# bgrozev/libjitsi

Measured on AMD Instinct MI355X. Metric: SRTP protect+unprotect packets/s + GB/s, 1200B AES_CM_128_HMAC_SHA1_80, 1-8 GPU, higher is better.
Workload: dtype u8; 1 GPU; configs[1]: 10k concurrent SSRCs x 1200-B RTP, AES_CM_128_HMAC_SHA1_80, protect + unprotect per step; ssrcs_per_gpu=10000, pkt_len=1200, region_align=16, ssrc_mix=round-robin, keysets=1, parallelism=ssrc-sharded x1 (one process per GPU), stream_events=device

## Files before the change

### libjitsi_amd/_native.py

```python
from __future__ import annotations

import ctypes as C
import os

import numpy as np

_HERE = os.path.dirname(os.path.abspath(__file__))
LIB_PATH = os.environ.get("SRTP_MI355X_LIB") or os.path.join(_HERE, "libsrtp_mi355x.so")
HEADER_PATH = os.path.join(os.path.dirname(_HERE), "include", "srtp_mi355x.h")

NULL_ENCRYPTION, AESCM_ENCRYPTION, AESF8_ENCRYPTION, TWOFISH_ENCRYPTION, TWOFISHF8_ENCRYPTION = range(5)
AESGCM_ENCRYPTION = 5
PROFILE_AEAD_AES_128_GCM, PROFILE_AEAD_AES_256_GCM = 0x0007, 0x0008
NULL_AUTHENTICATION, HMACSHA1_AUTHENTICATION = 0, 1
KIND_RTP, KIND_RTCP = 0, 1
(STATUS_OK, STATUS_DROP_REPLAY, STATUS_DROP_AUTH, STATUS_DROP_VERSION, STATUS_DROP_NO_CONTEXT,
 STATUS_ERR_CAPACITY, STATUS_ERR_MALFORMED, STATUS_DROP_INVALID, STATUS_NOT_PROCESSED,
 STATUS_SKIPPED, STATUS_ERR_INTERNAL) = range(11)
STATUS_NAMES = ["OK", "DROP_REPLAY", "DROP_AUTH", "DROP_VERSION", "DROP_NO_CONTEXT",
                "ERR_CAPACITY", "ERR_MALFORMED", "DROP_INVALID", "NOT_PROCESSED", "SKIPPED",
                "ERR_INTERNAL"]
NUM_STATUS = len(STATUS_NAMES)
DEBUG_FORCE_CHAIN_STALL = 0x1
DEBUG_FORCE_WIDE = 0x2
# ... 19 lines not shown
    "srtp_engine_last_error", "srtp_factory_create", "srtp_factory_close",
    "srtp_transformer_create", "srtp_transformer_set_factory", "srtp_transformer_close",
    "srtp_transform_device", "srtp_transform_host", "srtp_engine_sync",
    "srtp_get_context_state", "srtp_engine_num_contexts", "srtp_engine_set_timing",
    "srtp_engine_read_timing", "srtp_derive_session_keys", "srtp_export_contexts",
    "srtp_set_context_state", "srtp_pipeline_create", "srtp_pipeline_destroy",
    "srtp_pipeline_slot_get", "srtp_pipeline_submit", "srtp_pipeline_wait",
    "srtp_engine_stats", "srtp_engine_stream", "srtp_shard_of", "srtp_dispatch_plan", "srtp_dispatch_create",
    "srtp_dispatch_destroy", "srtp_dispatch_last_error", "srtp_dispatch_num_shards",
    "srtp_dispatch_engine", "srtp_dispatch_factory_create", "srtp_dispatch_factory_close",
    "srtp_dispatch_transformer_create", "srtp_dispatch_transformer_set_factory",
    "srtp_dispatch_transformer_close", "srtp_dispatch_transform_host", "srtp_dispatch_submit_host",
    "srtp_dispatch_wait_host",
    "srtp_dispatch_get_context_state", "srtp_dispatch_set_context_state", "srtp_dispatch_stats",
    "srtp_tls_export_keying_material", "srtp_dtls_profile_keys", "srtp_dtls_transformer_create",
    "srtp_engine_get_opts", "srtp_derive_session_keys_n", "srtp_derive_session_keys_for",
    "srtp_block_encrypt", "srtp_aes_gcm", "srtp_aggregator_opts_default", "srtp_aggregator_create",
    "srtp_aggregator_submit", "srtp_aggregator_flush", "srtp_aggregator_stats",
    "srtp_aggregator_destroy", "srtp_derive_session_keys_auth", "srtp_skein512_mac",
    "srtp_engine_set_debug", "srtp_contexts_save", "srtp_contexts_restore",
    "srtp_dispatch_route", "srtp_aggregator_create_dispatch", "srtp_transformer_info",
    "srtp_rawpacket_batch_create", "srtp_rawpacket_batch_create_dispatch",
    "srtp_rawpacket_batch_destroy", "srtp_rawpacket_transform", "srtp_rawpacket_result",
    "srtp_dispatch_host_times", "srtp_pipeline_submit_ex", "srtp_aggregator_transform",
    "srtp_aggregator_transformer_info", "srtp_rawpacket_transform_one", "srtp_device_count",
    "srtp_host_register", "srtp_host_unregister", "srtp_host_is_registered", "srtp_pipeline_submit_host",
    "srtp_pipeline_submit_gather",
    "srtp_pipeline_create_ex", "srtp_host_alloc", "srtp_host_free",
    "srtp_queue_create", "srtp_queue_submit", "srtp_queue_reap", "srtp_queue_outstanding",
    "srtp_queue_aggregator", "srtp_queue_destroy", "srtp_queue_release", "srtp_packet_may_throw",
    "srtp_rawpacket_batch_set_aggregator", "srtp_rawpacket_submit", "srtp_rawpacket_complete",
    "srtp_pipeline_query", "srtp_aes_gcm_device",
    "srtp_engine_enable_aead", "srtp_gcm_packet_job", "srtp_dtls_profile_keys_ex",
    "srtp_dispatch_enable_aead",
    "srtp_aes_gcm_device_ex", "srtp_gf128_mul", "srtp_gcm_hpowers", "srtp_gcm_wave_max",
    "srtp_small_aead_max",
    "srtp_trailer_room", "srtp_engine_trailer_room", "srtp_aggregator_trailer_room",
    "srtp_engine_gcm_stats", "srtp_dispatch_gcm_stats", "srtp_gcm_open_lane_min", "srtp_gcm_open_wave_min",
    "srtp_gcm_open_wave_max",
    "srtp_gcm_spec_ok", "srtp_gcm_fix_action",
    "srtp_fanout_device", "srtp_fanout_host", "srtp_engine_fanout_stats", "srtp_fanout_job",
    "srtp_fanout_device_rw", "srtp_fanout_host_rw", "srtp_fanout_rewrite_job",
    "srtp_fanout_device_ast", "srtp_fanout_host_ast", "srtp_fanout_ast_job",
    "srtp_fanout_device_pay", "srtp_fanout_host_pay", "srtp_fanout_pay_job",
    "srtp_transform_device_lvl", "srtp_transform_host_lvl", "srtp_engine_audio_level_stats",
    "srtp_audio_level_job",
    "srtp_fanout_device_red", "srtp_fanout_host_red", "srtp_engine_fanout_red_stats", "srtp_fanout_red_job",
    "srtp_fanout_device_fec", "srtp_fanout_host_fec", "srtp_engine_fanout_fec_stats", "srtp_fanout_fec_job",
]
STAGES = ["parse", "sort", "verify", "walk", "protect", "decrypt"]


KERNEL_SOURCES = ["srtp_kernels.hip", "aes_rounds_asm.inc", "srtp_kernels.h", "srtp_types.h", "engine.cpp",
                  "gcm_job.h", "fanout_job.h", "bundle_plan.h", "audio_level_job.h", "red_job.h", "fec_job.h"]


def kernel_source_sha16() -> str:
    import hashlib
    h = hashlib.sha256()
    for name in KERNEL_SOURCES:
        with open(os.path.join(_HERE, "csrc", name), "rb") as f:
            h.update(f.read())
    return h.hexdigest()[:16]


class SrtpError(RuntimeError):
    pass


class Policy(C.Structure):
    _fields_ = [(n, C.c_int32) for n in (
        "enc_type", "enc_key_len", "auth_type", "auth_key_len", "auth_tag_len", "salt_key_len")]


class EngineOpts(C.Structure):
    _fields_ = [("device", C.c_int32), ("check_replay", C.c_int32),
                ("abort_on_error", C.c_int32), ("max_contexts", C.c_uint32),
                ("max_factories", C.c_uint32), ("max_transformers", C.c_uint32),
                ("max_batch", C.c_uint32)]


class CtxState(C.Structure):
    _fields_ = [("roc", C.c_int32), ("s_l", C.c_int32), ("seq_num_set", C.c_int32),
                ("guessed_roc", C.c_int32), ("sent_index", C.c_int32),
                ("received_index", C.c_int32), ("replay_window", C.c_uint64),
                ("key_set", C.c_uint32)]


class Stats(C.Structure):
    _fields_ = ([("bundles", C.c_uint64), ("packets", C.c_uint64),
                 ("status", C.c_uint64 * NUM_STATUS)] +
                [(n, C.c_uint64) for n in ("roc_rechecks", "repaired", "ctx_overflow", "ctx_live",
                                           "ctx_tombstones", "ctx_slots", "rehashes", "chain_stalls", "long_walked",
                                           "holes", "small_bundles", "small_aead_bundles")])

    def as_dict(self) -> dict:
        d = {k: getattr(self, k) for k, _ in self._fields_ if k != "status"}
        d["status"] = {STATUS_NAMES[i]: int(self.status[i]) for i in range(NUM_STATUS)}
        return d


class DtlsKeys(C.Structure):
    _fields_ = [("srtp", Policy), ("srtcp", Policy), ("key_len", C.c_int32),
                ("salt_len", C.c_int32), ("keying_material_len", C.c_int32),
                ("client_key", C.c_uint8 * 16), ("server_key", C.c_uint8 * 16),
                ("client_salt", C.c_uint8 * 14), ("server_salt", C.c_uint8 * 14)]

# ... 358 lines not shown
```

### libjitsi_amd/csrc/srtp_kernels.hip

```cpp
#include <hip/hip_runtime.h>
#include <stdlib.h>
#include <string.h>

#include <algorithm>
#include <atomic>


#include "../../include/srtp_mi355x.h"
#include "audio_level_job.h"
#include "fanout_job.h"
#include "fec_job.h"
#include "gcm_job.h"
#include "red_job.h"
#include "srtp_kernels.h"

namespace srtp {

__device__ uint32_t d_te0[256];

constexpr int kBlock = 256;

__device__ __forceinline__ uint32_t rotl(uint32_t x, uint32_t n) {
    return __builtin_amdgcn_alignbit(x, x, 32u - n);
}
__device__ __forceinline__ uint32_t bswap(uint32_t x) { return __builtin_bswap32(x); }

__device__ __forceinline__ uint32_t ld_u8(const uint8_t *p) { return *p; }
__device__ __forceinline__ uint32_t ld_be32(const uint8_t *p) {
    return (ld_u8(p) << 24) | (ld_u8(p + 1) << 16) | (ld_u8(p + 2) << 8) | ld_u8(p + 3);
}

__device__ __forceinline__ uint64_t mix64(uint64_t x) {
    x ^= x >> 30; x *= 0xbf58476d1ce4e5b9ull;
    x ^= x >> 27; x *= 0x94d049bb133111ebull;
    x ^= x >> 31;
    return x;
}

__device__ __forceinline__ int32_t java_ishl1(int32_t n) { return (int32_t)(1u << (n & 31)); }
__device__ __forceinline__ int64_t java_lshl(int64_t v, int64_t n) {
    return (int64_t)((uint64_t)v << (n & 63));
}

constexpr int kTeWords = 32768;
constexpr int kTeCounters = 16;
constexpr int kAesBlock = 1024;
constexpr int kMacBlock = 256;
#ifndef SRTP_UNPROTECT_BLOCK
#define SRTP_UNPROTECT_BLOCK 1024
#endif
#ifndef SRTP_PROTECT_BLOCK
#define SRTP_PROTECT_BLOCK 1024
#endif
constexpr int kUnprotectBlock = SRTP_UNPROTECT_BLOCK;
constexpr int kProtectBlock = SRTP_PROTECT_BLOCK;

__device__ __forceinline__ void fill_te4(uint32_t *s_te) {
    const int W = (int)(blockDim.x >> 6), w = (int)(threadIdx.x >> 6), lane = (int)(threadIdx.x & 63u);
    const uint32_t r = (uint32_t)(lane >> 5) << 3;
    for (int j0 = 0; w + j0 * W < 256; j0 += 64) {
        const int ej = w + (j0 + lane) * W;
        const uint32_t mine = ej < 256 ? d_te0[ej] : 0u;
        for (int k = 0; k < 64; k++) {
            const int e = w + (j0 + k) * W;
            if (e >= 256) break;
            const uint32_t v = __builtin_amdgcn_readlane(mine, k);
            s_te[(e << 6) | lane] = rotl(v, r);
// ... 1932 lines not shown
    c.enc = ks->enc_type; c.auth = ks->auth_type; c.T = ks->tag_len; c.kind = ks->kind;
    c.check_replay = a.check_replay != 0;
    c.reverse = REV;
    const int32_t tid = (int32_t)(a.ctx_keys[slot] >> 32);
    const bool mac = c.auth != SRTP_NULL_AUTHENTICATION;
    uint32_t i = i0;
    uint32_t walked = 0u;
    for (;;) {
        const WalkRec *R = sm.rec;
        const uint32_t *G0 = sm.g0, *OK = sm.ok;
        int nvalid;
        if (pw) {
            const uint32_t jb = i - pw->base;
            int nv = 0;
#pragma unroll
            for (int k = 0; k < kLongPer; k++) {
                const uint32_t t = jb + (uint32_t)(lane + 64 * k);
                nv += (t < pw->win && pw->key[t] == key) ? 1 : 0;
            }
            nvalid = (int)__reduce_add_sync(~0ull, (unsigned)nv);
            R = pw->rec + jb; G0 = pw->g0 + jb; OK = pw->ok + jb;
        } else {
            int nv = 0;
#pragma unroll
            for (int k = 0; k < kLongPer; k++) {
                const int j = lane + 64 * k;
                const uint32_t idx = i + (uint32_t)j;
                const bool v = idx < a.n && a.sk_out[idx] == key;
                uint4 r = make_uint4(0u, 0u, 0u, 0u);
                if (v) r = reinterpret_cast<const uint4 *>(a.sv_out)[idx];
                reinterpret_cast<uint4 *>(sm.rec)[j] = r;
                if (REV) {
                    const uint32_t p = r.x & kRecIdxMask;
                    const uint2 go = v ? gok_of(a, p) : make_uint2(0u, 0u);
                    sm.g0[j] = go.x;
                    sm.ok[j] = go.y;
                }
                nv += v ? 1 : 0;
            }
            nvalid = (int)__reduce_add_sync(~0ull, (unsigned)nv);
            walk_sync();
        }
        if (nvalid == 0) break;
        int f = 0;
        if (c.kind == SRTP_KIND_RTP && (st.flags & 1u)) {
            const int p0 = lane * kLongPer;
            int32_t lsum = 0;
#pragma unroll 1
            for (int r = 0; r < kLongPer; r++) {
                const int pos = p0 + r;
                if (pos >= nvalid) break;
                const int32_t seq = (int32_t)(R[pos].word & 0xffffu);
                const int32_t sl = pos ? (int32_t)(R[pos - 1].word & 0xffffu) : st.b;
                int32_t d;
                if (sl < 32768) d = (seq - sl > 32768) ? -1 : 0;
                else d = (sl - 32768 > seq) ? 1 : 0;
                lsum += d;
            }
            uint32_t roc = (uint32_t)st.a + (uint32_t)wave_excl_scan(lsum);
            int first_bad = kLongPer;
#pragma unroll 1
            for (int r = 0; r < kLongPer; r++) {
                const int pos = p0 + r;
                if (pos >= nvalid) { first_bad = min(first_bad, r); break; }
                const WalkRec rec = R[pos];
                const int32_t seq = (int32_t)(rec.word & 0xffffu);
                const int32_t sl = pos ? (int32_t)(R[pos - 1].word & 0xffffu) : st.b;
                const uint32_t roc_prev = roc;
                int32_t d;
                if (sl < 32768) d = (seq - sl > 32768) ? -1 : 0;
                else d = (sl - 32768 > seq) ? 1 : 0;
                roc += (uint32_t)d;
                const int64_t delta = (java_lshl((int64_t)(int32_t)roc, 16) | (int64_t)seq) -
                                      (java_lshl((int64_t)(int32_t)roc_prev, 16) | (int64_t)sl);
                const int L = (int)(rec.lc & 0xffffu), C = (int)(rec.lc >> 16);
                bool g = delta > 0;
                if (REV) {
                    const int newL = mac ? (L - c.T > 0 ? L - c.T : 0) : L;
                    if (!(rec.p & kRecSkipDec)) g = g && !enc_would_throw(c.enc, rec.h, newL - rec.h);
                    if (g && mac) {
                        const uint32_t g0 = G0[pos], okb = OK[pos];
                        if (roc == g0) {
                            g = (okb & 1u) != 0u;
                        } else if ((okb & 4u) && roc == g0 - 1u) {
                            g = (okb & 2u) != 0u;
                        } else {
                            const uint32_t p = rec.p & kRecIdxMask;
                            ReverifyArgs rv;
                            rv.pkt = a.seg + a.off[p];
                            rv.mid = a.mid + 5 * (size_t)p;
                            rv.tailc = (a.spec[p] & kSpecDid) ? a.tailc + 16 * (size_t)p : nullptr;
                            g = reverify_tag<SK>(a, rv, ks, L, (int32_t)roc);
                        }
                    }
                } else {
                    g = g && L + (mac ? c.T : 0) <= C && !enc_would_throw(c.enc, rec.h, L - rec.h);
                }
                sm.roc[pos] = roc;
                sm.info[pos] = (g ? 1u : 0u) | ((uint32_t)((uint64_t)delta & 63u) << 1);
                if (!g) { first_bad = r; break; }
            }
            const unsigned long long bad_lanes = __ballot(first_bad < kLongPer);
            f = nvalid;
            if (bad_lanes) {
                const int bl = __ffsll((long long)bad_lanes) - 1;
                f = min(f, bl * kLongPer + __builtin_amdgcn_readlane(first_bad, bl));
            }
            int32_t dsum = 0;
            uint32_t recheck = 0u;
#pragma unroll 1
            for (int r = 0; r < kLongPer; r++) {
                const int pos = p0 + r;
                if (pos >= f) break;
                const WalkRec rec = R[pos];
                const uint32_t p = rec.p & kRecIdxMask;
                const int L = (int)(rec.lc & 0xffffu);
                const uint32_t rr = sm.roc[pos];
                a.w_cw[p] = rr;
                a.w_len[p] = (uint32_t)(REV ? (mac ? (L - c.T > 0 ? L - c.T : 0) : L) : L + (mac ? c.T : 0));
                a.w_status[p] = SRTP_STATUS_OK;
                if (REV && mac) {
                    const uint32_t g0 = G0[pos], okb = OK[pos];
                    if (rr != g0 && !((okb & 4u) && rr == g0 - 1u)) recheck++;
                }
                dsum += (int32_t)(sm.info[pos] >> 1);
            }
            if (f > 0) {
// ... 5 lines not shown
                    const int pos = p0 + r;
                    if (pos >= f) break;
                    after -= (int32_t)(sm.info[pos] >> 1);
                    if (after < 64) bits |= 1ull << after;
                }
                bits = wave_or64(bits);
                st.window = (total < 64 ? st.window << total : 0ull) | bits;
                st.a = (int32_t)sm.roc[f - 1];
                st.b = (int32_t)(R[f - 1].word & 0xffffu);
                st.g = st.a;
                const uint32_t rc = (uint32_t)__reduce_add_sync(~0ull, recheck);
                if (lane == 0 && rc) atomicAdd(&a.counters[kCtrRocRecheck], (unsigned long long)rc);
            }
        }
        walked += (uint32_t)(f < nvalid ? (c.kind == SRTP_KIND_RTP ? 1 : nvalid - f) : 0);
        if (f < nvalid) {
            const int stop = c.kind == SRTP_KIND_RTP ? f + 1 : nvalid;
            if (lane == 0) {
                for (int k = f; k < stop; k++) {
                    const WalkRec r = R[k];
                    uint32_t g0 = 0u, ok = 0u;
                    if (REV) { g0 = G0[k]; ok = OK[k]; }
                    (void)walk_one<SK>(a, ks, c, st, r, g0, ok, false, tid);
                }
            }
            bcast_state(st);
            i += (uint32_t)stop;
        } else {
            i += (uint32_t)nvalid;
        }
        walk_sync();
        if (nvalid < kLongStep && f >= nvalid) break;
    }
    if (lane == 0) {
        a.ctx[slot] = st;
        atomicAdd(&a.counters[kCtrLongWalked], (unsigned long long)walked);
    }
}

constexpr int kWalkBlock = 64;
#ifndef SRTP_WALK_PER
#define SRTP_WALK_PER 4
#endif
constexpr int kWalkPer = SRTP_WALK_PER;
constexpr int kWalkSpan = kWalkBlock * kWalkPer;
constexpr int kWalkAhead = 256;
constexpr int kWalkWin = kWalkSpan + kWalkAhead;
#ifndef SRTP_MED_MIN
#define SRTP_MED_MIN 32
#endif
constexpr uint32_t kMedMin = SRTP_MED_MIN;
constexpr int kMedMax = kWalkSpan / SRTP_MED_MIN + 1;
static_assert(kMedMax <= 64, "one medium chain start per lane");

constexpr int kChainPer = kWalkSpan / kWalkBlock;
static_assert(kLongMin == (uint32_t)kWalkSpan, "a long chain reaches the end of the tile it starts in");

struct ChainAgg {
    int32_t dsum;
    uint32_t x;
    uint32_t tshift;
    uint64_t bits;
    int32_t s_l;
    bool hasx, broken;
};
struct ChainState {
    uint32_t roc;
    int32_t s_l;
    uint64_t window;
    bool broken;
    bool stalled = false;
};

__device__ __forceinline__ ChainState chain_apply(ChainState p, const ChainAgg &g) {
    if (p.broken || g.broken || (g.hasx && p.roc != g.x) ||
        (int64_t)(int32_t)p.roc + g.dsum > (int64_t)0x7fffffff) {
        p.broken = true;
        return p;
    }
    p.roc += (uint32_t)g.dsum;
    p.s_l = g.s_l;
    p.window = (g.tshift < 64u ? p.window << g.tshift : 0ull) | g.bits;
    return p;
}

__device__ __forceinline__ ChainAgg chain_compose(const ChainAgg &g1, const ChainAgg &g2) {
    ChainAgg o;
    o.broken = g1.broken || g2.broken ||
               (g1.hasx && g2.hasx && g2.x - (uint32_t)g1.dsum != g1.x);
    o.dsum = g1.dsum + g2.dsum;
    o.hasx = g1.hasx || g2.hasx;
    o.x = g1.hasx ? g1.x : g2.x - (uint32_t)g1.dsum;
    o.tshift = min(g1.tshift + g2.tshift, 64u);
    o.bits = (g2.tshift < 64u ? g1.bits << g2.tshift : 0ull) | g2.bits;
    o.s_l = g2.s_l;
    return o;
}

constexpr int kLinkWords = 10;
__device__ __forceinline__ void gran_put(uint64_t *p, uint32_t epoch, uint32_t v) {
    __hip_atomic_store(p, ((uint64_t)v << 32) | epoch, __ATOMIC_RELAXED, __HIP_MEMORY_SCOPE_AGENT);
}
__device__ __forceinline__ bool gran_get(const uint64_t *p, uint32_t epoch, uint32_t &v) {
    const uint64_t g = __hip_atomic_load(p, __ATOMIC_RELAXED, __HIP_MEMORY_SCOPE_AGENT);
    v = (uint32_t)(g >> 32);
    return (uint32_t)g == epoch;
// ... 129 lines not shown
__device__ __forceinline__ void chain_window(const uint32_t m[kChainPer], int f, uint32_t &tshift,
                                             uint64_t &bits) {
    const int lane = (int)(threadIdx.x & 63u);
    int32_t msum = 0;
#pragma unroll
    for (int r = 0; r < kChainPer; r++)
        if (lane * kChainPer + r < f) msum += (int32_t)m[r];
    const int32_t total = (int32_t)__reduce_add_sync(~0ull, (unsigned)msum);
    int32_t after = total - wave_excl_scan(msum);
    uint64_t b = 0ull;
#pragma unroll
    for (int r = 0; r < kChainPer; r++) {
        if (lane * kChainPer + r < f) {
            after -= (int32_t)m[r];
            if (after < 64) b |= 1ull << after;
        }
    }
    bits = wave_or64(b);
    tshift = (uint32_t)min(total, 64);
}

struct ChainFix {
    uint32_t i0;
    CtxState st;
};

template <bool REV>
__device__ __forceinline__ ChainFix chain_part(const BundleArgs &a, uint32_t tile, uint32_t epoch, uint32_t base, uint32_t j0,
                               int n, bool head, bool out, int32_t prev_seq_in, const WalkRec *s_rec,
                               const uint32_t *s_g0, const uint32_t *s_ok) {
    ChainFix fix;
    fix.i0 = kNoSlot;
    const int lane = (int)(threadIdx.x & 63u);
    const uint32_t slot = a.sk_out[base + j0];
    const CtxState st0 = a.ctx[slot];
    const KeySet *ks = a.keysets + st0.ks;
    WalkCtx c;
    c.enc = ks->enc_type; c.auth = ks->auth_type; c.T = ks->tag_len; c.kind = ks->kind;
    const bool mac = c.auth != SRTP_NULL_AUTHENTICATION;
    const int32_t prev_seq = head ? st0.b : prev_seq_in;
    int32_t dpre[kChainPer];
    uint32_t m[kChainPer], xr[kChainPer];
    int32_t seqv[kChainPer];
    bool lok[kChainPer];
    int32_t lsum = 0;
#pragma unroll
    for (int r = 0; r < kChainPer; r++) {
        const int pos = lane * kChainPer + r;
        dpre[r] = 0; m[r] = 0u; xr[r] = 0u; seqv[r] = 0; lok[r] = false;
        if (pos >= n) continue;
        const WalkRec rec = s_rec[j0 + pos];
        const int32_t seq = (int32_t)(rec.word & 0xffffu);
        const int32_t sl = pos ? (int32_t)(s_rec[j0 + pos - 1].word & 0xffffu) : prev_seq;
        int32_t d;
        if (sl < 32768) d = (seq - sl > 32768) ? -1 : 0;
        else d = (sl - 32768 > seq) ? 1 : 0;
        const int64_t delta = (int64_t)d * 65536 + seq - sl;
        const int L = (int)(rec.lc & 0xffffu), C = (int)(rec.lc >> 16);
        bool ok = delta > 0;
        if (REV) {
            const int newL = mac ? (L - c.T > 0 ? L - c.T : 0) : L;
            if (!(rec.p & kRecSkipDec)) ok = ok && !enc_would_throw(c.enc, rec.h, newL - rec.h);
            if (mac) ok = ok && (s_ok[j0 + pos] & 1u) != 0u;
        } else {
            ok = ok && L + (mac ? c.T : 0) <= C && !enc_would_throw(c.enc, rec.h, L - rec.h);
        }
        lok[r] = ok;
        lsum += d;
        dpre[r] = lsum;
        m[r] = (uint32_t)((uint64_t)delta & 63u);
        seqv[r] = seq;
    }
    const int32_t dex = wave_excl_scan(lsum);
#pragma unroll
    for (int r = 0; r < kChainPer; r++) {
        dpre[r] += dex;
        if (REV && mac && lane * kChainPer + r < n) xr[r] = s_g0[j0 + lane * kChainPer + r] - (uint32_t)dpre[r];
    }
    const bool hasx = REV && mac && n > 0;
    const uint32_t x0 = (uint32_t)__builtin_amdgcn_readfirstlane((int)xr[0]);
    int fb = kChainPer;
#pragma unroll
    for (int r = kChainPer - 1; r >= 0; r--)
        if (lane * kChainPer + r < n && (!lok[r] || (hasx && xr[r] != x0))) fb = r;
    int first_bad = n;
    {
        const unsigned long long bl = __ballot(fb < kChainPer);
        if (bl) {
            const int l = __ffsll((long long)bl) - 1;
            first_bad = l * kChainPer + __builtin_amdgcn_readlane(fb, l);
        }
    }
    auto at = [&](const int32_t v[kChainPer], int pos) -> int32_t {
        int32_t x = 0;
#pragma unroll
        for (int r = 0; r < kChainPer; r++)
            if (pos % kChainPer == r) x = __builtin_amdgcn_readlane(v[r], pos / kChainPer);
        return x;
    };
    if (out && !head) {
        ChainAgg g;
        chain_window(m, first_bad, g.tshift, g.bits);
        g.dsum = first_bad ? at(dpre, first_bad - 1) : 0;
        g.s_l = first_bad ? at(seqv, first_bad - 1) : 0;
        g.x = x0;
        g.hasx = hasx;
        g.broken = first_bad < n;
        chain_publish_agg(a, tile, epoch, g);
    }
// ... 48 lines not shown
    }
    CtxState cs = st0;
    cs.a = (int32_t)st.roc; cs.b = st.s_l; cs.g = (int32_t)g_out; cs.window = st.window;
    if (f < n) {
        fix.i0 = base + j0 + (uint32_t)f;
        fix.st = cs;
        st.broken = true;
        if (out) chain_publish_state(a, tile, epoch, st);
        return fix;
    }
    if (out) chain_publish_state(a, tile, epoch, st);
    else if (lane == 0) a.ctx[slot] = cs;
    return fix;
}

__device__ __forceinline__ ChainFix chain_stall_next(const BundleArgs &a, uint32_t epoch, uint32_t &t) {
    ChainFix f;
    f.i0 = kNoSlot;
    for (; t < gridDim.x; t++) {
        uint32_t i0 = 0u;
        const bool st = gran_get(a.tile_link + (size_t)t * kLinkWords + 9, epoch, i0);
        if (!__builtin_amdgcn_readfirstlane((int)st)) continue;
        uint32_t v[4];
        bool pr = true;
#pragma unroll
        for (int i = 0; i < 4; i++) {
            pr &= gran_get(a.tile_link + (size_t)(t - 1u) * kLinkWords + 5 + i, epoch, v[i]);
            v[i] = (uint32_t)__builtin_amdgcn_readfirstlane((int)v[i]);
        }
        if (!__builtin_amdgcn_readfirstlane((int)pr) || (v[1] & 0x10000u)) continue;
        i0 = (uint32_t)__builtin_amdgcn_readfirstlane((int)i0);
        f.st = a.ctx[a.sk_out[i0]];
        f.st.a = (int32_t)v[0];
        f.st.b = (int32_t)(v[1] & 0xffffu);
        f.st.g = f.st.a;
        f.st.window = (uint64_t)v[2] | ((uint64_t)v[3] << 32);
        f.i0 = i0;
        t++;
        return f;
    }
    return f;
}


template <bool REV>
struct WalkShared {
    WalkRec rec[kWalkWin];
    uint32_t key[kWalkWin];
    uint32_t g0[REV ? kWalkWin : 1];
    uint32_t ok[REV ? kWalkWin : 1];
    uint32_t start[kWalkSpan > kLongStep ? kWalkSpan : kLongStep];
    uint32_t pkey[kWalkSpan];
    uint32_t med[kMedMax];
    uint32_t nstart, tile, nmed;
};
static_assert(kLongStep <= kWalkWin, "walk_long stages a step in the first pass's arrays");
static_assert(kLongStep <= kWalkSpan, "a medium chain's walk_long step keeps its ROCs in s_pkey");

template <bool GCM>
__device__ __forceinline__ bool gcm_slot(const BundleArgs &a, uint32_t key) {
    if constexpr (GCM) return key <= a.ctx_mask && a.keysets[a.ctx[key].ks].pad == kGcmMark;
    else return false;
}

template <bool REV, bool SK, int PASS, bool GCM = false>
__device__ __forceinline__ void walk_tile(const BundleArgs &a, WalkShared<REV> &sh, uint32_t blk, uint32_t nblk) {
    constexpr int limit_pass = PASS;
    WalkRec *const s_rec = sh.rec;
    uint32_t *const s_key = sh.key;
    uint32_t *const s_g0 = sh.g0;
    uint32_t *const s_ok = sh.ok;
    uint32_t *const s_start = sh.start;
    uint32_t &s_nstart = sh.nstart;
    uint32_t *const s_pkey = sh.pkey;
    uint32_t &s_tile = sh.tile;
    uint32_t *const s_med = sh.med;
    uint32_t &s_nmed = sh.nmed;
    const bool two_pass = a.abort_on_error && a.ctl->any_throw;
    const bool chains = !two_pass;
    const bool chain_pass = limit_pass && !two_pass;
    if (chain_pass && a.ctl->n_long == 0u) return;
    if (!limit_pass) {
        for (uint32_t i = blk * kWalkBlock + threadIdx.x; i < a.sort_zero_words; i += nblk * kWalkBlock)
            a.sort_zero[i] = 0u;
        for (uint32_t i = blk * kWalkBlock + threadIdx.x; i < a.sort_zero_words / 256u * kClsWords;
             i += nblk * kWalkBlock)
            a.cls_tile[i] = 0u;
    }
    uint32_t tile = blk;
    if (chain_pass) {
        if (threadIdx.x == 0) s_tile = atomicAdd(&a.ctl->tile_ticket, 1u);
        walk_sync();
        tile = s_tile;
    }
    const uint32_t base = tile * kWalkSpan;
    if (base >= a.n) return;
    const uint32_t span = min((uint32_t)kWalkSpan, a.n - base);
    const uint32_t win = min((uint32_t)kWalkWin, a.n - base);
    if (threadIdx.x == 0) { s_nstart = 0; s_nmed = 0; }
    if (chain_pass && base) {
#pragma unroll
        for (int k = 0; k < kWalkPer; k++) {
            const uint32_t j = threadIdx.x + k * kWalkBlock;
            s_pkey[j] = a.sk_out[base - kWalkSpan + j];
        }
    }
#pragma unroll
    for (int k = 0; k < kWalkWin / kWalkBlock; k++) {
        const uint32_t j = threadIdx.x + k * kWalkBlock;
        if (j < win) {
            const WalkRec r = a.sv_out[base + j];
            const uint32_t key = a.sk_out[base + j];
            s_rec[j] = r;
            s_key[j] = key;
            if (REV && key <= a.ctx_mask) {
                const uint32_t p = r.p & kRecIdxMask;
                const uint2 go = gok_of(a, p);
                s_g0[j] = go.x;
                s_ok[j] = go.y;
            }
        }
    }
    walk_sync();
    const uint32_t prev_key = base ? a.sk_out[base - 1] : ~0u;
    auto long_from = [&](uint32_t j, uint32_t key) -> bool {
        const uint32_t jl = j + kLongMin - 1u;
        const uint32_t kl = jl < win ? s_key[jl] : (base + jl < a.n ? a.sk_out[base + jl] : ~0u);
        return kl == key;
    };
    if constexpr (PASS == 1) if (chain_pass) {
        const uint32_t epoch = a.serial + 1u;
        uint32_t key0 = s_key[0];
        if constexpr (GCM)
            if (gcm_slot<true>(a, key0)) key0 = kNoSlot;
        bool in_long = false;
        if (base && key0 == prev_key && key0 <= a.ctx_mask) {
            if (s_pkey[0] == key0) {
                in_long = true;
            } else {
                uint32_t sj = kWalkSpan;
#pragma unroll
                for (int k = 0; k < kWalkPer; k++) {
                    const uint32_t j = threadIdx.x * kWalkPer + k;
                    if (s_pkey[j] == key0 && (j == 0 || s_pkey[j - 1] != key0)) sj = j;
                }
                sj = (uint32_t)__reduce_min_sync(~0ull, sj);
                in_long = sj > 0 && sj < (uint32_t)kWalkSpan && s_key[sj - 1] == key0;
            }
        }
        uint32_t keyl = s_key[span - 1];
        if constexpr (GCM)
            if (gcm_slot<true>(a, keyl)) keyl = kNoSlot;
// ... 32 lines not shown
        sm.rec = s_rec;
        sm.roc = s_key;
        sm.g0 = REV ? s_g0 : s_start;
        sm.ok = REV ? s_ok : s_start;
        sm.info = s_start;
        uint32_t t_fix = 1u;
        bool fixup = false;
#pragma unroll 1
        for (int q = 0;; q++) {
            ChainFix f;
            if (q == 0) {
                f = fix_in;
            } else if (q == 1) {
                f = fix_head;
            } else {
                if (q == 2) {
                    uint32_t last = 0u;
                    if (threadIdx.x == 0) {
                        __threadfence();
                        last = atomicAdd(&a.ctl->tiles_done, 1u) == nblk - 1u ? 1u : 0u;
                        if (last) {
                            __threadfence();
                            last = __hip_atomic_load(&a.ctl->n_stall, __ATOMIC_RELAXED,
                                                     __HIP_MEMORY_SCOPE_AGENT) != 0u ? 1u : 0u;
                        }
                    }
                    fixup = __builtin_amdgcn_readfirstlane((int)last) != 0;
                }
                if (!fixup) break;
                f = chain_stall_next(a, epoch, t_fix);
                if (f.i0 == kNoSlot) break;
            }
            if (f.i0 != kNoSlot) walk_long<REV, SK>(a, f.i0, sm, f.st);
        }
        return;
    }
#pragma unroll
    for (int k = 0; k < kWalkPer; k++) {
        const uint32_t j = threadIdx.x + k * kWalkBlock;
        if (j < span) {
            const uint32_t key = s_key[j];
            if (key <= a.ctx_mask && (j ? s_key[j - 1] : prev_key) != key)
                s_start[atomicAdd(&s_nstart, 1u)] = j;
        }
    }
    walk_sync();
    const uint32_t nstart = s_nstart;
    const bool dry = two_pass && !limit_pass;
#pragma unroll 1
    for (uint32_t q = threadIdx.x; q < nstart; q += kWalkBlock) {
        const uint32_t j = s_start[q];
        const uint32_t key = s_key[j];
        const uint32_t slot = key;
        if constexpr (GCM) {
            if (gcm_slot<true>(a, key)) {
                CtxState st = a.ctx[slot];
                const uint32_t ks_id = st.ks;
                const KeySet *ks = a.keysets + ks_id;
                WalkCtx c;
                c.enc = ks->enc_type; c.auth = ks->auth_type; c.T = ks->tag_len; c.kind = ks->kind;
                c.check_replay = a.check_replay != 0;
                c.reverse = REV;
                const int32_t tid = (int32_t)(a.ctx_keys[slot] >> 32);
                const int32_t E = limit_pass ? a.e_min[tid] : 0x7fffffff;
                const uint32_t first_p = s_rec[j].p & kRecIdxMask;
                bool more = true;
                uint32_t jj = j;
                for (; jj < win && more; jj++) {
                    if (s_key[jj] != key) { more = false; break; }
                    const WalkRec r = s_rec[jj];
                    if (limit_pass && (int32_t)(r.p & kRecIdxMask) > E) { more = false; break; }
                    more = walk_one_gcm(a, ks_id, slot, c, st, r, REV ? s_g0[jj] : 0u, REV ? s_ok[jj] : 0u, dry, tid);
                }
                for (uint32_t i = base + jj; more && i < a.n; i++) {
                    if (a.sk_out[i] != key) break;
                    const WalkRec r = a.sv_out[i];
                    if (limit_pass && (int32_t)(r.p & kRecIdxMask) > E) break;
                    uint32_t g0 = 0u, ok = 0u;
                    if (REV) {
                        const uint2 go = gok_of(a, r.p & kRecIdxMask);
                        g0 = go.x; ok = go.y;
                    }
                    more = walk_one_gcm(a, ks_id, slot, c, st, r, g0, ok, dry, tid);
                }
                if (dry) continue;
                if (limit_pass && st.birth == a.serial && (int32_t)first_p > E) {
                    __hip_atomic_store(&a.ctx_keys[slot], kTombKey, __ATOMIC_RELAXED, __HIP_MEMORY_SCOPE_AGENT);
                    continue;
                }
                a.ctx[slot] = st;
                continue;
            }
        }
        if (chains && long_from(j, key)) {
            atomicOr(&a.ctl->n_long, 1u);
            continue;
        }
        if (chains && j + kMedMin - 1u < win && s_key[j + kMedMin - 1u] == key) {
            s_med[atomicAdd(&s_nmed, 1u)] = j;
            continue;
        }
        CtxState st = a.ctx[slot];
        const KeySet *ks = a.keysets + st.ks;
        WalkCtx c;
        c.enc = ks->enc_type; c.auth = ks->auth_type; c.T = ks->tag_len; c.kind = ks->kind;
        c.check_replay = a.check_replay != 0;
        c.reverse = REV;
        const int32_t tid = (int32_t)(a.ctx_keys[slot] >> 32);
        const int32_t E = limit_pass ? a.e_min[tid] : 0x7fffffff;
        const uint32_t first_p = s_rec[j].p & kRecIdxMask;
        auto step = [&](const WalkRec &r, uint32_t g0, uint32_t ok) -> bool {
            if (limit_pass && (int32_t)(r.p & kRecIdxMask) > E) return false;
            return walk_one<SK>(a, ks, c, st, r, g0, ok, dry, tid);
        };
        uint32_t jj = j;
        if (!two_pass && c.kind == SRTP_KIND_RTP && (st.flags & 1u)) {
            const bool mac = c.auth != SRTP_NULL_AUTHENTICATION;
            for (; jj < win; jj++) {
                if (s_key[jj] != key) break;
                const WalkRec rec = s_rec[jj];
                const int32_t seq = (int32_t)(rec.word & 0xffffu);
                const int32_t sl = st.b;
                int32_t d;
                if (sl < 32768) d = (seq - sl > 32768) ? -1 : 0;
                else d = (sl - 32768 > seq) ? 1 : 0;
                const uint32_t g = (uint32_t)st.a + (uint32_t)d;
                const int64_t delta = (java_lshl((int64_t)(int32_t)g, 16) | (int64_t)seq) -
                                      (java_lshl((int64_t)st.a, 16) | (int64_t)sl);
                const int L = (int)(rec.lc & 0xffffu), C = (int)(rec.lc >> 16);
                bool keep = delta > 0;
                int newL;
                if (REV) {
                    newL = mac ? (L - c.T > 0 ? L - c.T : 0) : L;
                    if (!(rec.p & kRecSkipDec)) keep = keep && !enc_would_throw(c.enc, rec.h, newL - rec.h);
                    if (mac) {
                        const uint32_t g0 = s_g0[jj], okb = s_ok[jj];
                        keep = keep && (g == g0 ? (okb & 1u) != 0u
                                                : (okb & 4u) != 0u && g == g0 - 1u && (okb & 2u) != 0u);
                    }
                } else {
                    newL = L + (mac ? c.T : 0);
                    keep = keep && newL <= C && !enc_would_throw(c.enc, rec.h, L - rec.h);
                }
                if (!keep) break;
                const uint32_t p = rec.p & kRecIdxMask;
                a.w_cw[p] = g;
                a.w_len[p] = (uint32_t)newL;
                a.w_status[p] = SRTP_STATUS_OK;
                st.window = (uint64_t)java_lshl((int64_t)st.window, delta) | 1ull;
                st.a = (int32_t)g;
                st.b = seq;
                st.g = (int32_t)g;
            }
        }
        bool more = true;
        for (; jj < win; jj++) {
            if (s_key[jj] != key) { more = false; break; }
            if (!step(s_rec[jj], REV ? s_g0[jj] : 0u, REV ? s_ok[jj] : 0u)) { more = false; break; }
        }
        for (uint32_t i = base + jj; more && i < a.n; i++) {
            if (a.sk_out[i] != key) break;
            const WalkRec r = a.sv_out[i];
            uint32_t g0 = 0u, ok = 0u;
            if (REV) {
                const uint32_t p = r.p & kRecIdxMask;
                const uint2 go = gok_of(a, p);
                g0 = go.x; ok = go.y;
            }
            if (!step(r, g0, ok)) break;
        }
        if (dry) continue;
        if (limit_pass && st.birth == a.serial && (int32_t)first_p > E) {
            __hip_atomic_store(&a.ctx_keys[slot], kTombKey, __ATOMIC_RELAXED, __HIP_MEMORY_SCOPE_AGENT);
            continue;
        }
        a.ctx[slot] = st;
    }
    if (!chains) return;
    walk_sync();
    const uint32_t nmed = s_nmed;
    if (nmed == 0u) return;
    uint32_t med = threadIdx.x < nmed ? s_med[threadIdx.x] : 0u;
    LongWin pw;
    pw.rec = s_rec;
    pw.key = s_key;
    pw.g0 = REV ? s_g0 : s_start;
    pw.ok = REV ? s_ok : s_start;
    pw.base = base;
    pw.win = win;
    LongLds sm;
    sm.rec = s_rec;
    sm.roc = s_pkey;
    sm.g0 = REV ? s_g0 : s_start;
    sm.ok = REV ? s_ok : s_start;
    sm.info = s_start;
    walk_sync();
#pragma unroll 1
    for (uint32_t m = 0; m < nmed; m++) {
        const uint32_t j = (uint32_t)__builtin_amdgcn_readlane((int)med, (int)m);
        const CtxState st = a.ctx[s_key[j]];
        walk_long<REV, SK>(a, base + j, sm, st, &pw);
    }
}

template <bool REV, bool SK, int PASS, bool GCM = false>
__global__ __launch_bounds__(kWalkBlock) void k_walk(BundleArgs a) {
    __shared__ WalkShared<REV> sh;
// ... 3819 lines not shown
```

Measured before the change: 372.8 million packets/s.

## Replace serial short-chain SRTP walk with wave-wide segmented prefix scan

Short per-SSRC chains in the walk tile were advanced one thread per chain, serially walking each packet's ROC and replay window. This adds a segmented parallel scan across the wave that computes the ROC, index delta and 64-bit replay window for every record in the tile at once. Records that fail or lack a fast-path context are queued, with their partial state, to the existing serial walker. The aim is to remove serial per-chain latency and load imbalance, at the cost of extra shared memory (four scan arrays per tile, which may lower occupancy) and more shuffles.

```diff
diff --git a/libjitsi_amd/_native.py b/libjitsi_amd/_native.py
--- a/libjitsi_amd/_native.py
+++ b/libjitsi_amd/_native.py
@@ -95,7 +95,8 @@
 
 
 KERNEL_SOURCES = ["srtp_kernels.hip", "aes_rounds_asm.inc", "srtp_kernels.h", "srtp_types.h", "engine.cpp",
-                  "gcm_job.h", "fanout_job.h", "bundle_plan.h", "audio_level_job.h", "red_job.h", "fec_job.h"]
+                  "gcm_job.h", "fanout_job.h", "bundle_plan.h", "audio_level_job.h", "red_job.h", "fec_job.h",
+                  "walk_prefix.h"]
 
 
 def kernel_source_sha16() -> str:
diff --git a/libjitsi_amd/csrc/srtp_kernels.hip b/libjitsi_amd/csrc/srtp_kernels.hip
--- a/libjitsi_amd/csrc/srtp_kernels.hip
+++ b/libjitsi_amd/csrc/srtp_kernels.hip
@@ -13,6 +13,7 @@
 #include "gcm_job.h"
 #include "red_job.h"
 #include "srtp_kernels.h"
+#include "walk_prefix.h"
 
 namespace srtp {
 
@@ -2051,10 +2052,7 @@
                 if (pos >= nvalid) break;
                 const int32_t seq = (int32_t)(R[pos].word & 0xffffu);
                 const int32_t sl = pos ? (int32_t)(R[pos - 1].word & 0xffffu) : st.b;
-                int32_t d;
-                if (sl < 32768) d = (seq - sl > 32768) ? -1 : 0;
-                else d = (sl - 32768 > seq) ? 1 : 0;
-                lsum += d;
+                lsum += wp_step(seq, sl);
             }
             uint32_t roc = (uint32_t)st.a + (uint32_t)wave_excl_scan(lsum);
             int first_bad = kLongPer;
@@ -2066,12 +2064,8 @@
                 const int32_t seq = (int32_t)(rec.word & 0xffffu);
                 const int32_t sl = pos ? (int32_t)(R[pos - 1].word & 0xffffu) : st.b;
                 const uint32_t roc_prev = roc;
-                int32_t d;
-                if (sl < 32768) d = (seq - sl > 32768) ? -1 : 0;
-                else d = (sl - 32768 > seq) ? 1 : 0;
-                roc += (uint32_t)d;
-                const int64_t delta = (java_lshl((int64_t)(int32_t)roc, 16) | (int64_t)seq) -
-                                      (java_lshl((int64_t)(int32_t)roc_prev, 16) | (int64_t)sl);
+                roc += (uint32_t)wp_step(seq, sl);
+                const int64_t delta = wp_delta(roc, seq, roc_prev, sl);
                 const int L = (int)(rec.lc & 0xffffu), C = (int)(rec.lc >> 16);
                 bool g = delta > 0;
                 if (REV) {
@@ -2183,6 +2177,13 @@
 constexpr uint32_t kMedMin = SRTP_MED_MIN;
 constexpr int kMedMax = kWalkSpan / SRTP_MED_MIN + 1;
 static_assert(kMedMax <= 64, "one medium chain start per lane");
+constexpr int kScanPer = (kWalkSpan + (int)kMedMin - 1 + kWalkBlock - 1) / kWalkBlock;
+constexpr int kScanLen = kWalkBlock * kScanPer;
+static_assert(kWalkSpan + (int)kMedMin - 1 <= kScanLen && kScanLen <= kWalkWin, "the scan covers every short chain");
+constexpr uint32_t kWpValid = 0x80000000u;
+constexpr uint32_t kWpMac = 0x40000000u;
+constexpr int kWpEncShift = 24;
+constexpr int kWpTagShift = 16;
 
 constexpr int kChainPer = kWalkSpan / kWalkBlock;
 static_assert(kLongMin == (uint32_t)kWalkSpan, "a long chain reaches the end of the tile it starts in");
@@ -2418,9 +2419,7 @@
         const WalkRec rec = s_rec[j0 + pos];
         const int32_t seq = (int32_t)(rec.word & 0xffffu);
         const int32_t sl = pos ? (int32_t)(s_rec[j0 + pos - 1].word & 0xffffu) : prev_seq;
-        int32_t d;
-        if (sl < 32768) d = (seq - sl > 32768) ? -1 : 0;
-        else d = (sl - 32768 > seq) ? 1 : 0;
+        const int32_t d = wp_step(seq, sl);
         const int64_t delta = (int64_t)d * 65536 + seq - sl;
         const int L = (int)(rec.lc & 0xffffu), C = (int)(rec.lc >> 16);
         bool ok = delta > 0;
@@ -2575,7 +2574,9 @@
     uint32_t start[kWalkSpan > kLongStep ? kWalkSpan : kLongStep];
     uint32_t pkey[kWalkSpan];
     uint32_t med[kMedMax];
-    uint32_t nstart, tile, nmed;
+    uint32_t c_roc[kScanLen], c_prop[kScanLen], c_wlo[kScanLen], c_whi[kScanLen];
+    uint32_t ser[kWalkSpan];
+    uint32_t nstart, tile, nmed, nser;
 };
 static_assert(kLongStep <= kWalkWin, "walk_long stages a step in the first pass's arrays");
 static_assert(kLongStep <= kWalkSpan, "a medium chain's walk_long step keeps its ROCs in s_pkey");
@@ -2584,6 +2585,156 @@
 __device__ __forceinline__ bool gcm_slot(const BundleArgs &a, uint32_t key) {
     if constexpr (GCM) return key <= a.ctx_mask && a.keysets[a.ctx[key].ks].pad == kGcmMark;
     else return false;
+}
+
+template <bool REV>
+__device__ __forceinline__ void walk_scan(const BundleArgs &a, WalkShared<REV> &sh, uint32_t span, uint32_t win,
+                                          uint32_t prev_key) {
+    const int lane = (int)(threadIdx.x & 63u);
+    const uint32_t p0 = (uint32_t)lane * kScanPer;
+    const WalkRec *const s_rec = sh.rec;
+    const uint32_t *const s_key = sh.key;
+    constexpr uint32_t kHeadBit = 0x20000000u;
+    uint32_t keyv[kScanPer + 1];
+    int32_t seqv[kScanPer], prevv[kScanPer];
+    uint32_t gv[kScanPer], propv[kScanPer];
+    bool headv[kScanPer], seen[kScanPer];
+    WpSum run;
+    run.g = 0u; run.prop = 0u; run.head = false;
+    {
+        const bool pv = p0 && p0 - 1u < win;
+        uint32_t kprev = p0 ? (pv ? s_key[p0 - 1u] : kNoSlot) : prev_key;
+        int32_t sprev = pv ? (int32_t)(s_rec[p0 - 1u].word & 0xffffu) : 0;
+#pragma unroll
+        for (int r = 0; r < kScanPer; r++) {
+            const uint32_t pos = p0 + (uint32_t)r;
+            const bool valid = pos < win;
+            const uint32_t key = valid ? s_key[pos] : kNoSlot;
+            const int32_t seq = valid ? (int32_t)(s_rec[pos].word & 0xffffu) : 0;
+            const bool head = !valid || key != kprev;
+            const bool own = head && valid && pos < span && key <= a.ctx_mask;
+            WpSum e;
+            e.prop = own ? sh.c_prop[pos] : 0u;
+            const int32_t prev = head ? (int32_t)(e.prop & 0xffffu) : sprev;
+            e.g = (own ? sh.c_roc[pos] : 0u) + (uint32_t)wp_step(seq, prev);
+            e.head = head;
+            run = wp_sum(run, e);
+            keyv[r] = key; seqv[r] = seq; prevv[r] = prev; headv[r] = head;
+            gv[r] = run.g; propv[r] = run.prop; seen[r] = run.head;
+            kprev = key; sprev = seq;
+        }
+        const uint32_t pn = p0 + (uint32_t)kScanPer;
+        keyv[kScanPer] = pn < win ? s_key[pn] : kNoSlot;
+    }
+    WpSum ex;
+    {
+        WpSum inc = run;
+#pragma unroll
+        for (int o = 1; o < 64; o <<= 1) {
+            WpSum y;
+            y.g = (uint32_t)__shfl_up((int)inc.g, o, 64);
+            const uint32_t w = (uint32_t)__shfl_up((int)(inc.prop | (inc.head ? kHeadBit : 0u)), o, 64);
+            y.prop = w & ~kHeadBit;
+            y.head = (w & kHeadBit) != 0u;
+            if (lane >= o) inc = wp_sum(y, inc);
+        }
+        ex.g = (uint32_t)__shfl_up((int)inc.g, 1, 64);
+        ex.prop = (uint32_t)__shfl_up((int)inc.prop, 1, 64);
+        ex.head = false;
+        if (lane == 0) { ex.g = 0u; ex.prop = 0u; }
+    }
+    uint32_t pv_[kScanPer], lenv[kScanPer], ev[kScanPer];
+    WpWin agg;
+    agg.shift = 0u; agg.bits = 0ull; agg.bad = false; agg.head = false;
+    auto win_elem = [&](int r, uint32_t pos) -> WpWin {
+        const bool keep = (ev[r] & 64u) != 0u;
+        const bool first = headv[r] && (propv[r] & kWpValid);
+        if (first) return wp_win_first((uint64_t)sh.c_wlo[pos] | ((uint64_t)sh.c_whi[pos] << 32), (int64_t)(ev[r] & 63u), keep);
+        return wp_win_rec((int64_t)(ev[r] & 63u), keep, headv[r]);
+    };
+#pragma unroll
+    for (int r = 0; r < kScanPer; r++) {
+        const uint32_t pos = p0 + (uint32_t)r;
+        if (!seen[r]) { gv[r] += ex.g; propv[r] += ex.prop; }
+        const uint32_t prop = propv[r];
+        pv_[r] = 0u; lenv[r] = 0u; ev[r] = 0u;
+        if (prop & kWpValid) {
+            const WalkRec rec = s_rec[pos];
+            const uint32_t g = gv[r];
+            const uint32_t g_prev = headv[r] ? sh.c_roc[pos] : (r ? gv[r ? r - 1 : 0] : ex.g);
+            const int64_t delta = wp_delta(g, seqv[r], g_prev, prevv[r]);
+            const bool mac = (prop & kWpMac) != 0u;
+            const int enc = (int)((prop >> kWpEncShift) & 0xfu), T = (int)((prop >> kWpTagShift) & 0xffu);
+            const int L = (int)(rec.lc & 0xffffu), C = (int)(rec.lc >> 16);
+            bool keep = delta > 0;
+            int newL;
+            if (REV) {
+                newL = mac ? (L - T > 0 ? L - T : 0) : L;
+                if (!(rec.p & kRecSkipDec)) keep = keep && !enc_would_throw(enc, rec.h, newL - rec.h);
+                if (mac) {
+                    const uint32_t g0 = sh.g0[pos], okb = sh.ok[pos];
+                    keep = keep && (g == g0 ? (okb & 1u) != 0u
+                                            : (okb & 4u) != 0u && g == g0 - 1u && (okb & 2u) != 0u);
+                }
+            } else {
+                newL = L + (mac ? T : 0);
+                keep = keep && newL <= C && !enc_would_throw(enc, rec.h, L - rec.h);
+            }
+            pv_[r] = rec.p & kRecIdxMask;
+            lenv[r] = (uint32_t)newL;
+            ev[r] = (uint32_t)((uint64_t)delta & 63u) | (keep ? 64u : 0u);
+        }
+        agg = wp_win(agg, win_elem(r, pos));
+    }
+    WpWin run2;
+    {
+        WpWin inc = agg;
+#pragma unroll
+        for (int o = 1; o < 64; o <<= 1) {
+            WpWin y;
+            const uint32_t w = (uint32_t)__shfl_up((int)(inc.shift | (inc.bad ? 0x100u : 0u) | (inc.head ? 0x200u : 0u)), o, 64);
+            const uint32_t lo = (uint32_t)__shfl_up((int)(uint32_t)inc.bits, o, 64);
+            const uint32_t hi = (uint32_t)__shfl_up((int)(uint32_t)(inc.bits >> 32), o, 64);
+            y.shift = w & 0xffu; y.bad = (w & 0x100u) != 0u; y.head = (w & 0x200u) != 0u;
+            y.bits = (uint64_t)lo | ((uint64_t)hi << 32);
+            if (lane >= o) inc = wp_win(y, inc);
+        }
+        const uint32_t w = (uint32_t)__shfl_up((int)(inc.shift | (inc.bad ? 0x100u : 0u)), 1, 64);
+        const uint32_t lo = (uint32_t)__shfl_up((int)(uint32_t)inc.bits, 1, 64);
+        const uint32_t hi = (uint32_t)__shfl_up((int)(uint32_t)(inc.bits >> 32), 1, 64);
+        run2.shift = w & 0xffu; run2.bad = (w & 0x100u) != 0u; run2.head = false;
+        run2.bits = (uint64_t)lo | ((uint64_t)hi << 32);
+        if (lane == 0) { run2.shift = 0u; run2.bits = 0ull; run2.bad = false; }
+    }
+#pragma unroll
+    for (int r = 0; r < kScanPer; r++) {
+        const uint32_t pos = p0 + (uint32_t)r;
+        const WpWin before = run2;
+        run2 = wp_win(run2, win_elem(r, pos));
+        if (!(propv[r] & kWpValid)) continue;
+        if (!headv[r] && before.bad) continue;
+        if (ev[r] & 64u) {
+            const uint32_t p = pv_[r];
+            a.w_cw[p] = gv[r];
+            a.w_len[p] = lenv[r];
+            a.w_status[p] = SRTP_STATUS_OK;
+            if (keyv[r + 1] != keyv[r]) {
+                CtxState *cs = a.ctx + keyv[r];
+                cs->a = (int32_t)gv[r];
+                cs->b = seqv[r];
+                cs->g = (int32_t)gv[r];
+                cs->window = run2.bits;
+            }
+        } else {
+            sh.ser[atomicAdd(&sh.nser, 1u)] = pos;
+            if (!headv[r]) {
+                sh.c_roc[pos] = r ? gv[r ? r - 1 : 0] : ex.g;
+                sh.c_prop[pos] = (uint32_t)prevv[r];
+                sh.c_wlo[pos] = (uint32_t)before.bits;
+                sh.c_whi[pos] = (uint32_t)(before.bits >> 32);
+            }
+        }
+    }
 }
 
 template <bool REV, bool SK, int PASS, bool GCM = false>
@@ -2620,7 +2771,7 @@
     if (base >= a.n) return;
     const uint32_t span = min((uint32_t)kWalkSpan, a.n - base);
     const uint32_t win = min((uint32_t)kWalkWin, a.n - base);
-    if (threadIdx.x == 0) { s_nstart = 0; s_nmed = 0; }
+    if (threadIdx.x == 0) { s_nstart = 0; s_nmed = 0; sh.nser = 0; }
     if (chain_pass && base) {
 #pragma unroll
         for (int k = 0; k < kWalkPer; k++) {
@@ -2759,6 +2910,7 @@
         const uint32_t j = s_start[q];
         const uint32_t key = s_key[j];
         const uint32_t slot = key;
+        sh.c_prop[j] = 0u;
         if constexpr (GCM) {
             if (gcm_slot<true>(a, key)) {
                 CtxState st = a.ctx[slot];
@@ -2807,7 +2959,40 @@
             s_med[atomicAdd(&s_nmed, 1u)] = j;
             continue;
         }
+        if constexpr (PASS == 0) if (!two_pass) {
+            const CtxState st = a.ctx[slot];
+            const KeySet *ks = a.keysets + st.ks;
+            const int enc = ks->enc_type, auth = ks->auth_type, T = ks->tag_len, kind = ks->kind;
+            if (kind == SRTP_KIND_RTP && (st.flags & 1u) && (uint32_t)st.b <= 0xffffu) {
+                sh.c_roc[j] = (uint32_t)st.a;
+                sh.c_wlo[j] = (uint32_t)st.window;
+                sh.c_whi[j] = (uint32_t)(st.window >> 32);
+                sh.c_prop[j] = kWpValid | (auth != SRTP_NULL_AUTHENTICATION ? kWpMac : 0u) |
+                               (((uint32_t)enc & 0xfu) << kWpEncShift) | (((uint32_t)T & 0xffu) << kWpTagShift) |
+                               (uint32_t)st.b;
+                continue;
+            }
+        }
+        sh.ser[atomicAdd(&sh.nser, 1u)] = j;
+    }
+    if constexpr (PASS == 0) if (!two_pass) {
+        walk_sync();
+        walk_scan<REV>(a, sh, span, win, prev_key);
+    }
+    walk_sync();
+    const uint32_t nser = sh.nser;
+#pragma unroll 1
+    for (uint32_t q = threadIdx.x; q < nser; q += kWalkBlock) {
+        const uint32_t j = sh.ser[q];
+        const uint32_t key = s_key[j];
+        const uint32_t slot = key;
         CtxState st = a.ctx[slot];
+        if ((j ? s_key[j - 1] : prev_key) == key) {
+            st.a = (int32_t)sh.c_roc[j];
+            st.b = (int32_t)sh.c_prop[j];
+            st.g = st.a;
+            st.window = (uint64_t)sh.c_wlo[j] | ((uint64_t)sh.c_whi[j] << 32);
+        }
         const KeySet *ks = a.keysets + st.ks;
         WalkCtx c;
         c.enc = ks->enc_type; c.auth = ks->auth_type; c.T = ks->tag_len; c.kind = ks->kind;
@@ -2821,45 +3006,6 @@
             return walk_one<SK>(a, ks, c, st, r, g0, ok, dry, tid);
         };
         uint32_t jj = j;
-        if (!two_pass && c.kind == SRTP_KIND_RTP && (st.flags & 1u)) {
-            const bool mac = c.auth != SRTP_NULL_AUTHENTICATION;
-            for (; jj < win; jj++) {
-                if (s_key[jj] != key) break;
-                const WalkRec rec = s_rec[jj];
-                const int32_t seq = (int32_t)(rec.word & 0xffffu);
-                const int32_t sl = st.b;
-                int32_t d;
-                if (sl < 32768) d = (seq - sl > 32768) ? -1 : 0;
-                else d = (sl - 32768 > seq) ? 1 : 0;
-                const uint32_t g = (uint32_t)st.a + (uint32_t)d;
-                const int64_t delta = (java_lshl((int64_t)(int32_t)g, 16) | (int64_t)seq) -
-                                      (java_lshl((int64_t)st.a, 16) | (int64_t)sl);
-                const int L = (int)(rec.lc & 0xffffu), C = (int)(rec.lc >> 16);
-                bool keep = delta > 0;
-                int newL;
-                if (REV) {
-                    newL = mac ? (L - c.T > 0 ? L - c.T : 0) : L;
-                    if (!(rec.p & kRecSkipDec)) keep = keep && !enc_would_throw(c.enc, rec.h, newL - rec.h);
-                    if (mac) {
-                        const uint32_t g0 = s_g0[jj], okb = s_ok[jj];
-                        keep = keep && (g == g0 ? (okb & 1u) != 0u
-                                                : (okb & 4u) != 0u && g == g0 - 1u && (okb & 2u) != 0u);
-                    }
-                } else {
-                    newL = L + (mac ? c.T : 0);
-                    keep = keep && newL <= C && !enc_would_throw(c.enc, rec.h, L - rec.h);
-                }
-                if (!keep) break;
-                const uint32_t p = rec.p & kRecIdxMask;
-                a.w_cw[p] = g;
-                a.w_len[p] = (uint32_t)newL;
-                a.w_status[p] = SRTP_STATUS_OK;
-                st.window = (uint64_t)java_lshl((int64_t)st.window, delta) | 1ull;
-                st.a = (int32_t)g;
-                st.b = seq;
-                st.g = (int32_t)g;
-            }
-        }
         bool more = true;
         for (; jj < win; jj++) {
             if (s_key[jj] != key) { more = false; break; }
diff --git a/libjitsi_amd/csrc/walk_prefix.h b/libjitsi_amd/csrc/walk_prefix.h
--- /dev/null
+++ b/libjitsi_amd/csrc/walk_prefix.h
@@ -0,0 +1,77 @@
+#pragma once
+#include <stdint.h>
+
+#if defined(__HIPCC__) || defined(__CUDACC__)
+#define SRTP_WP_HD __host__ __device__ __forceinline__
+#else
+#define SRTP_WP_HD inline
+#endif
+
+namespace srtp {
+
+SRTP_WP_HD int32_t wp_step(int32_t seq, int32_t prev) {
+    if (prev < 32768) return (seq - prev > 32768) ? -1 : 0;
+    return (prev - 32768 > seq) ? 1 : 0;
+}
+
+SRTP_WP_HD int64_t wp_index(uint32_t g, int32_t seq) {
+    return (int64_t)((uint64_t)(int64_t)(int32_t)g << 16) | (int64_t)seq;
+}
+
+SRTP_WP_HD int64_t wp_delta(uint32_t g, int32_t seq, uint32_t g_prev, int32_t prev) {
+    return wp_index(g, seq) - wp_index(g_prev, prev);
+}
+
+struct WpSum {
+    uint32_t g;
+    uint32_t prop;
+    bool head;
+};
+
+SRTP_WP_HD WpSum wp_sum(const WpSum &l, const WpSum &r) {
+    if (r.head) return r;
+    WpSum o;
+    o.g = l.g + r.g;
+    o.prop = l.prop + r.prop;
+    o.head = l.head;
+    return o;
+}
+
+struct WpWin {
+    uint32_t shift;
+    uint64_t bits;
+    bool bad;
+    bool head;
+};
+
+SRTP_WP_HD WpWin wp_win_rec(int64_t delta, bool keep, bool head) {
+    WpWin o;
+    o.shift = (uint32_t)((uint64_t)delta & 63u);
+    o.bits = 1ull;
+    o.bad = !keep;
+    o.head = head;
+    return o;
+}
+
+SRTP_WP_HD WpWin wp_win_first(uint64_t window, int64_t delta, bool keep) {
+    WpWin o;
+    const uint32_t m = (uint32_t)((uint64_t)delta & 63u);
+    o.shift = 64u;
+    o.bits = (window << m) | 1ull;
+    o.bad = !keep;
+    o.head = true;
+    return o;
+}
+
+SRTP_WP_HD WpWin wp_win(const WpWin &l, const WpWin &r) {
+    if (r.head) return r;
+    WpWin o;
+    const uint32_t s = l.shift + r.shift;
+    o.shift = s < 64u ? s : 64u;
+    o.bits = (r.shift < 64u ? l.bits << r.shift : 0ull) | r.bits;
+    o.bad = l.bad || r.bad;
+    o.head = l.head;
+    return o;
+}
+
+}
```

Measured after the change: 373.7 million packets/s, median of 6. About the same (+0.2%).
